# zyansheep/shadow

Hardware: AMD Instinct MI355X
Metric: APSP routing build (s) @10k nodes; packets routed/sec per sim round (lower is better)
Workload: dtype u64+f32; 1 GPU; C3 APSP routing build: 10k-node undirected ring+chords graph, mean degree 8, latency U[1,100] ms (integer us), loss 0 w.p. 0.8 else U(0,0.02); all nodes used; source rows sharded across ranks (each rank keeps its row block; the optional RCCL all-gather of the blocks is timed separately in apsp_detail.allgather_ms); nodes=10000, arcs=79996, parallelism=rows1

## Files before the change

### shadow_amd/csrc/sg_internal.h

```cpp
#pragma once

#include <hip/hip_runtime.h>

#include <cstdint>
#include <cstdio>
#include <new>
#include <stdexcept>
#include <string>
#include <atomic>
#include <deque>
#include <memory>
#include <vector>

#include "../../include/shadow_gpu.h"

namespace sg {

struct Error : std::runtime_error {
  int32_t code;
  uint32_t row, col;
  Error(int32_t c, const std::string& m, uint32_t r = 0, uint32_t k = 0)
      : std::runtime_error(m), code(c), row(r), col(k) {}
};

// ... 182 lines not shown
}

constexpr uint32_t SB_SUB = 8;
constexpr uint32_t SB_CTL_STRIDE = SB_SUB * 4096 + 1;

inline unsigned grid_for(size_t n, unsigned block, unsigned cap = 1u << 20) {
  size_t g = (n + block - 1) / block;
  if (g == 0) g = 1;
  if (g > cap) g = cap;
  return (unsigned)g;
}

void exclusive_scan_u32(sg_ctx* ctx, const uint32_t* d_in, uint32_t* d_out, uint32_t n);

void launch_group_offsets(sg_ctx* ctx, const uint32_t* key, uint32_t n, uint32_t n_groups, uint32_t* off,
                          uint32_t* err);

void copy_to_host(sg_ctx* ctx, void* dst, const void* src, size_t bytes);

char* stage_acquire(sg_ctx* ctx, int slot, size_t bytes);
void stage_release(sg_ctx* ctx, int slot);

void timer_add_work(sg_ctx* ctx, const char* name, double work);
void timer_set_counter(sg_ctx* ctx, const char* name, double work, uint64_t n);

struct TimedLaunch {
  sg_ctx* ctx;
  KernelTimer* timer = nullptr;
  hipEvent_t e0 = nullptr, e1 = nullptr;
  TimedLaunch(sg_ctx* c, const char* name, double work);
  ~TimedLaunch();
};

constexpr uint32_t DENSE_MAX = 4096;
bool sssp_dense_fits(uint32_t n_nodes);
void launch_sssp_dense(sg_ctx* ctx, sg_net* net, const uint32_t* d_used, uint32_t n_used, uint32_t row_begin,
                       uint32_t row_end, uint64_t* out_lat, float* out_loss, uint32_t* sat_row,
                       unsigned long long* work);

bool sssp_bucket_fits(uint32_t n_nodes);
void launch_sssp_bucket(sg_ctx* ctx, sg_net* net, const uint32_t* d_used, uint32_t n_used, uint32_t row_begin,
                        uint32_t row_end, uint64_t* out_lat, float* out_loss, uint32_t* sat_row,
                        unsigned long long* work, unsigned long long* diag);

constexpr int SSSP_KB_MAX = 8;
constexpr uint32_t SSSP_UB_EXACT = 0x80000000u;
bool sssp_lds_fits(uint32_t n_nodes);

struct SsspChainDesc {
  uint32_t* claim;
  const uint32_t* rel;
  const uint8_t* phase_of;
  const uint32_t* pos;
  uint32_t exact, check_rows;
};

struct SsspLdsLaunch {
  const uint32_t* d_used = nullptr;
  uint32_t n_used = 0, row_begin = 0, row_end = 0;
  uint64_t* out_lat = nullptr;
  float* out_loss = nullptr;
  uint32_t* sat_row = nullptr;
  uint32_t delta = 0;
  unsigned long long* work = nullptr;
  unsigned long long* diag = nullptr;
  const uint32_t* blk_rows = nullptr;
  uint32_t n_blk = 0;
  const uint32_t* ub_row = nullptr;
  const uint32_t* ub_w = nullptr;
  const uint32_t* plan_ctl = nullptr;
  int plan_ph = 0;
  uint32_t* plan_ctr = nullptr;
  uint32_t* done = nullptr;
  const SsspChainDesc* chain = nullptr;
};
void launch_sssp_lds(sg_ctx* ctx, const sg_net* net, const SsspLdsLaunch& l);

void ensure_csc(sg_ctx* ctx, sg_net* net);
std::string node_name(const sg_net* net, uint32_t idx);
void launch_zero2(sg_ctx* ctx, uint32_t* a, uint32_t na, uint32_t* b, uint32_t nb);

constexpr int WORK_SHARDS = 64;
void shortest_paths_slab(sg_ctx* ctx, sg_net* net, const uint32_t* d_used, uint32_t n_used, uint32_t row_begin,
                         uint32_t row_end, uint64_t* out_lat, float* out_loss);
void run_wide(sg_ctx* ctx, sg_net* net, const uint32_t* d_used, uint32_t n_used, const std::vector<uint32_t>& rows,
              uint32_t out_row0, uint64_t* out_lat, float* out_loss);

struct SsspDevPlan {
  int n_phase = 0;
  uint32_t* list = nullptr;
  uint32_t* ub_row = nullptr;
  uint32_t* ub_w = nullptr;
  uint32_t* ctl = nullptr;
  uint32_t* ctr = nullptr;
  const SsspChainDesc* chain = nullptr;
  bool landmarks = false;
  unsigned rows_grid = 0;
};
constexpr int SSSP_PHASES_MAX = 6;
SsspDevPlan sssp_device_plan(sg_ctx* ctx, sg_net* net, const uint32_t* d_used, uint32_t n_used, uint32_t row_begin,
                             uint32_t row_end, int n_phase, int kb, bool exact, int hops, uint32_t n_land,
                             uint32_t* zero_rows = nullptr, uint32_t* zero_rows2 = nullptr, bool chain = false,
                             bool chain_exact = false);
const SsspChainDesc* sssp_plain_rel(sg_ctx* ctx, const sg_net* net, const uint32_t* d_used, uint32_t row_begin,
                                    uint32_t row_end, uint32_t* zero_rows, uint32_t* claim, uint32_t* zero_ctr,
                                    bool chain_exact);
void sssp_landmark_bounds(sg_ctx* ctx, const SsspDevPlan& p, uint32_t n_used, uint32_t row_begin,
                          const uint64_t* out_lat, const uint32_t* sat_row, int kb);

}
```

### shadow_amd/csrc/sg_plan.hip

```cpp
#include <algorithm>
#include <cstdlib>
#include <vector>

#include "sg_device.h"
#include "sg_internal.h"
#include "sg_knobs.h"

namespace sg {

__global__ void k_plan_rel(const uint32_t* __restrict__ used, uint32_t row_begin, uint32_t rows,
                           uint32_t* __restrict__ rel, uint8_t* __restrict__ jn, uint32_t* __restrict__ zero_rows,
                           uint32_t* __restrict__ zero_rows2, uint32_t* __restrict__ zero_ctr,
                           SsspChainDesc* __restrict__ desc, SsspChainDesc desc_val) {
  const uint32_t r = blockIdx.x * blockDim.x + threadIdx.x;
  if (zero_ctr && r < 2) zero_ctr[r] = 0;
  if (desc && r == 0) *desc = desc_val;
  if (r >= rows) return;
  rel[used[row_begin + r]] = r;
  if (jn) jn[r] = 0;
  if (zero_rows) zero_rows[r] = 0;
  if (zero_rows2) zero_rows2[r] = 0;
}

constexpr uint32_t PL_OOB = 0x80000000u;
// ... 346 lines not shown
    const uint32_t m = min<uint32_t>(fcnt[wv][cur], PB_FMAX);
    if (!m) break;
    uint32_t carry = 0;
    for (uint32_t e0 = 0; e0 < m; e0 += 64) {
      const uint32_t e = e0 + lane;
      const uint32_t d = e < m ? out_off[fx[wv][cur][e] + 1] - out_off[fx[wv][cur][e]] : 0u;
      const uint32_t incl = wave_incl_sum(d);
      if (e < m) fpre[wv][e] = carry + incl - d;
      carry += __builtin_amdgcn_readlane(incl, 63);
    }
    if (lane == 0) {
      fpre[wv][m] = carry;
      fcnt[wv][cur ^ 1] = 0;
    }
    __builtin_amdgcn_fence(__ATOMIC_RELEASE, "wavefront");
    __builtin_amdgcn_wave_barrier();
    __builtin_amdgcn_fence(__ATOMIC_ACQUIRE, "wavefront");
    for (uint32_t tt = lane; tt < carry; tt += 64) {
      uint32_t lo = 0, hi = m;
      while (hi - lo > 1) {
        const uint32_t mid = (lo + hi) / 2;
        if (fpre[wv][mid] <= tt) lo = mid;
        else hi = mid;
      }
      visit(out_off[fx[wv][cur][lo]] + (tt - fpre[wv][lo]), fw[wv][cur][lo], level, cur ^ 1);
    }
    cur ^= 1;
  }
  for (int k = 0; k < kb; k++) {
    uint64_t mk = t[0];
    for (int d = 32; d > 0; d >>= 1) mk = min(mk, (uint64_t)__shfl_xor((unsigned long long)mk, d));
    if (mk == ~0ull) break;
    const uint32_t q = (uint32_t)mk & 0x7FFFFFFFu;
    if (lane == 0) {
      orow[k] = (row_begin + q) | ((mk >> 63) ? 0u : SSSP_UB_EXACT);
      ow[k] = (uint32_t)(mk >> 31);
    }
#pragma unroll
    for (int j = 0; j < PB_LIST; j++)
      if (((uint32_t)t[j] & 0x7FFFFFFFu) == q) t[j] = ~0ull;
#pragma unroll
    for (int p = 0; p < PB_LIST; p++)
#pragma unroll
      for (int j = 0; j + 1 < PB_LIST; j++) {
        const uint64_t lo = min(t[j], t[j + 1]), hi = max(t[j], t[j + 1]);
        t[j] = lo;
        t[j + 1] = hi;
      }
  }
}

SsspDevPlan sssp_device_plan(sg_ctx* ctx, sg_net* net, const uint32_t* d_used, uint32_t n_used, uint32_t row_begin,
                             uint32_t row_end, int n_phase, int kb, bool exact, int hops, uint32_t n_land,
                             uint32_t* zero_rows, uint32_t* zero_rows2, bool chain, bool chain_exact) {
  (void)n_used;
  const uint32_t n = net->n_nodes, rows = row_end - row_begin;
  n_phase = std::max(2, std::min(SSSP_PHASES_MAX - (n_land ? 1 : 0), n_phase));
  const size_t nl = rows, nb = (size_t)rows * SSSP_KB_MAX;
  const size_t words = nl + 2 * nb + 4 * SSSP_PHASES_MAX + n + 2 * (size_t)rows + 2 * ((rows + 3) / 4) +
                       (sizeof(SsspChainDesc) + 8) / 4;
  uint32_t* w = ctx->r_plan.get<uint32_t>(words);
  SsspDevPlan p;
  p.n_phase = n_phase;
  p.list = w;
  p.ub_row = p.list + nl;
  p.ub_w = p.ub_row + nb;
  p.ctl = p.ub_w + nb;
  p.ctr = p.ctl + 2 * SSSP_PHASES_MAX;
  uint32_t* rel = p.ctr + 2 * SSSP_PHASES_MAX;
  uint32_t* gain = rel + n;
  uint32_t* pos = gain + rows;
  uint8_t* jn = (uint8_t*)(pos + rows);
  uint8_t* phase_of = jn + (rows + 3) / 4 * 4;
  SsspChainDesc* desc = (SsspChainDesc*)(((uintptr_t)(phase_of + (rows + 3) / 4 * 4) + 7) & ~(uintptr_t)7);
  const SsspChainDesc desc_val{zero_rows2, rel, phase_of, pos, chain_exact ? 1u : 0u, 0u};
  if (chain) p.chain = desc;
  hipStream_t st = ctx->stream;
  {
    TimedLaunch tl(ctx, "plan_sets", 0.0);
    if (rows != n) SG_HIP(hipMemsetAsync(rel, 0xff, (size_t)n * 4, st));
    const unsigned g = grid_for(rows, 256);
    hipLaunchKernelGGL(k_plan_rel, dim3(g), dim3(256), 0, st, d_used, row_begin, rows, rel, jn, zero_rows, zero_rows2,
                       (uint32_t*)nullptr, chain ? desc : (SsspChainDesc*)nullptr, desc_val);
    if (net->directed) ensure_csc(ctx, net);
    const uint32_t* in_off = net->directed ? net->in_off : net->out_off;
    const uint32_t* in_idx = net->directed ? net->in_src : net->out_arc;
    const uint32_t in_stride = net->directed ? 1u : 3u;
    for (int ph = 0; ph + 1 < n_phase; ph++) {
      hipLaunchKernelGGL(k_vote_gain, dim3(g), dim3(256), 0, st, in_off, in_idx, in_stride, d_used, row_begin, rows,
                         rel, jn, gain);
      hipLaunchKernelGGL(k_vote_name, dim3(g), dim3(256), 0, st, net->out_off, net->out_arc, d_used, row_begin, rows,
                         rel, jn, gain, ph);
    }
    if (n_land) {
      hipLaunchKernelGGL(k_plan_landmarks<1024>, dim3(1), dim3(1024), 0, st, jn, rows, n_land);
      n_phase += 1;
      p.n_phase = n_phase;
      p.landmarks = true;
      p.rows_grid = grid_for(rows, 256);
    }
    hipLaunchKernelGGL(k_plan_lists<1024>, dim3(1), dim3(1024), 0, st, jn, rows, row_begin, n_phase, phase_of, p.list,
                       pos, p.ctl, p.ctr);
    SG_CHECK_LAUNCH();
  }
  {
    TimedLaunch tl(ctx, "plan_bounds", 0.0);
    hipLaunchKernelGGL(k_plan_bounds, dim3((rows + PB_WAVES - 1) / PB_WAVES), dim3(PB_WAVES * 64), 0, ctx->stream,
                       net->out_off, net->out_arc, d_used, rel, phase_of, p.list, rows, row_begin,
                       std::max(1, std::min(SSSP_KB_MAX, kb)), exact ? 1 : 0, std::max(1, std::min(3, hops)),
                       p.ub_row, p.ub_w);
    SG_CHECK_LAUNCH();
  }
  if (knob_int("SG_PLAN_DIAG", 0) != 0) {
    uint32_t h[2 * SSSP_PHASES_MAX];
    copy_to_host(ctx, h, p.ctl, sizeof(h));
    fprintf(stderr, "[plan] %u rows:", rows);
    for (int ph = 0; ph < n_phase; ph++) fprintf(stderr, " %u", h[2 * ph + 1]);
    fprintf(stderr, "\n");
  }
  return p;
}

const SsspChainDesc* sssp_plain_rel(sg_ctx* ctx, const sg_net* net, const uint32_t* d_used, uint32_t row_begin,
                                    uint32_t row_end, uint32_t* zero_rows, uint32_t* claim, uint32_t* zero_ctr,
                                    bool chain_exact) {
  const uint32_t n = net->n_nodes, rows = row_end - row_begin;
  const size_t dw = sizeof(SsspChainDesc) / 4;
  uint32_t* w = ctx->r_plan.get<uint32_t>(dw + n);
  SsspChainDesc* desc = (SsspChainDesc*)w;
  uint32_t* rel = w + dw;
  const SsspChainDesc desc_val{claim, rel, nullptr, nullptr, chain_exact ? 1u : 0u, rows != n ? rows : 0u};
  hipLaunchKernelGGL(k_plan_rel, dim3(grid_for(rows, 256)), dim3(256), 0, ctx->stream, d_used, row_begin, rows, rel,
                     (uint8_t*)nullptr, zero_rows, claim, zero_ctr, desc, desc_val);
  SG_CHECK_LAUNCH();
  return desc;
}

}
```

### shadow_amd/csrc/sg_routing.hip

```cpp
#include <algorithm>
#include <cstring>
#include <string>
#include <vector>

#include "sg_device.h"
#include "sg_internal.h"
#include "sg_knobs.h"

namespace sg {

__global__ void k_self_check(const uint32_t* __restrict__ used, uint32_t n_used,
                             const uint32_t* __restrict__ self_cnt,
                             unsigned long long* __restrict__ first) {
  for (uint32_t j = blockIdx.x * blockDim.x + threadIdx.x; j < n_used; j += gridDim.x * blockDim.x) {
    uint32_t c = self_cnt[used[j]];
    if (c != 1) atomicMin(first, ((unsigned long long)j << 1) | (c > 1 ? 1ull : 0ull));
  }
}

__global__ void __launch_bounds__(1024) k_build_finish(const uint32_t* __restrict__ sat, uint32_t rows,
                                                       const uint32_t* __restrict__ used, uint32_t n_used,
                                                       const uint32_t* __restrict__ self_cnt, uint32_t* __restrict__ ret) {
  constexpr int G = 8;
  __shared__ uint32_t s_cnt[16];
// ... 231 lines not shown
}

static void print_bucket_diag(const sg_net* net, uint32_t rows, const unsigned long long* d, double total) {
  const double nb = std::max(1.0, (double)d[0]);
  fprintf(stderr, "[bucket] %u rows: %.1f buckets, %.0f entries, %.2f far steps, %.0f pops in %.0f claims, "
          "%.0f relaxations (%.3f x arcs) per row\n", rows, d[0] / (double)rows, d[1] / (double)rows,
          d[2] / (double)rows, d[3] / (double)rows, d[8] / (double)rows, total / rows,
          total / rows / std::max(1u, net->n_arcs));
  fprintf(stderr, "[bucket] cycles per bucket (thread 0): phase 0 %.0f, phase 1 %.0f, phase 2 %.0f; output per row %.0f\n",
          d[4] / nb, d[5] / nb, d[6] / nb, d[7] / (double)rows);
  fprintf(stderr, "[bucket] band kernel, wave 0 per bucket: offsets %.0f, arcs (with appends) %.0f, appends %.0f, store wait %.0f; "
          "band splits per row %.2f\n", d[9] / nb, d[10] / nb, d[11] / nb, d[12] / nb, d[15] / (double)rows);
  fprintf(stderr, "[bucket] band kernel, thread 0 per bucket in the load step: entry loads %.0f, hash %.0f, barrier wait %.0f\n",
          d[8] / nb, d[13] / nb, d[14] / nb);
  const double ncl = std::max(1.0, (double)d[8]);
  fprintf(stderr, "[bucket] per wave and bucket: load step %.0f cyc, idle %.0f; per claim: to offsets %.0f, to "
          "arcs %.0f (sum over arc rounds), appends %.0f, claim total %.0f\n", d[9] / nb / 4, d[14] / nb / 4,
          d[10] / ncl, d[11] / ncl, d[12] / ncl, d[13] / ncl);
}

static void shortest_paths_bucket(sg_ctx* ctx, sg_net* net, const uint32_t* d_used, uint32_t n_used,
                                  uint32_t row_begin, uint32_t row_end, uint64_t* out_lat, float* out_loss) {
  const bool diag_on = knob_int("SG_BUCKET_DIAG", 0) != 0;
  const uint32_t rows = row_end - row_begin;
  uint32_t* sat = ctx->r_flags.get<uint32_t>(std::max(rows, 1u));
  SG_HIP(hipMemsetAsync(sat, 0, std::max(rows, 1u) * 4ull, ctx->stream));
  unsigned long long* work = ctx->count_work ? ctx->r_work.get<unsigned long long>(WORK_SHARDS + 16) : nullptr;
  unsigned long long* diag = work ? work + WORK_SHARDS : nullptr;
  if (work) SG_HIP(hipMemsetAsync(work, 0, (WORK_SHARDS + 16) * 8, ctx->stream));
  {
    TimedLaunch tl(ctx, "sssp_bucket", 0.0);
    launch_sssp_bucket(ctx, net, d_used, n_used, row_begin, row_end, out_lat, out_loss, sat, work, diag);
  }
  std::vector<uint32_t> wide_rows = finish_rows(ctx, sat, row_begin, rows);
  if (work) {
    unsigned long long w[WORK_SHARDS + 16];
    const double total = read_work(ctx, work, w, 16);
    timer_add_work(ctx, "sssp_bucket", total);
    timer_add_work(ctx, "sssp_bucket_entries", (double)w[WORK_SHARDS + 1]);
    if (diag_on) print_bucket_diag(net, rows, w + WORK_SHARDS, total);
  }
  if (!wide_rows.empty()) run_wide(ctx, net, d_used, n_used, wide_rows, row_begin, out_lat, out_loss);
}

struct LdsKnobs {
  uint32_t delta;
  bool diag;
  bool flagged;
  bool phased;
  int n_phase, kb, hops;
  bool exact;
  uint32_t n_land;
  bool chain;
};
static LdsKnobs lds_knobs(const sg_ctx* ctx, const sg_net* net, uint32_t n_used, uint32_t rows) {
  LdsKnobs k;
  k.delta = (uint32_t)std::min(4294967295.0, std::max(1.0, knob_double("SG_APSP_DELTA", 4294967295.0)));
  k.diag = knob_int("SG_SSSP_DIAG", 0) != 0;
  const int seeds_env = knob_int("SG_SSSP_SEEDS", 1);
  const int flag_env = knob_int("SG_SSSP_FLAGGED", -1);
  const bool few_rows = rows < 6u * (uint32_t)std::max(1, ctx->n_cu);
  k.flagged = seeds_env != 0 && (flag_env == 1 || (flag_env < 0 && rows < n_used && !few_rows));
  k.phased = !k.flagged && seeds_env != 0 && (seeds_env == 2 || rows >= 8u * (uint32_t)ctx->n_cu);
  const bool chain = !knob_off("SG_SSSP_CHAIN") && !net->directed && !k.flagged;
  const uint32_t per_cu = rows / std::max(1, ctx->n_cu);
  k.n_phase = knob_int("SG_SSSP_PHASES", per_cu >= 16 && !chain ? 3 : 2, 2, SSSP_PHASES_MAX);
  k.kb = knob_int("SG_SSSP_BOUNDS", 2, 1, SSSP_KB_MAX);
  k.exact = knob_int("SG_SSSP_EXACT", 1) != 0 && n_used == net->n_nodes;
  k.hops = knob_int("SG_SSSP_HOPS", 3, 1, 3);
  const int land_env = knob_int("SG_SSSP_LANDMARKS", 0);
  k.n_land = net->directed || land_env <= 0 ? 0u : (uint32_t)land_env;
  k.chain = chain;
  return k;
}

static void print_sssp_diag(sg_ctx* ctx, const sg_net* net, const unsigned long long* diag, uint32_t n_diag,
                            uint32_t delta) {
  std::vector<unsigned long long> h((size_t)n_diag * 8);
  copy_to_host(ctx, h.data(), diag, h.size() * 8);
  double a[8] = {0, 0, 0, 0, 0, 0, 0, 0};
  double setup = 0;
  double cn[2] = {0, 0}, cs[2] = {0, 0}, cq[2] = {0, 0};
  for (uint32_t r = 0; r < n_diag; r++) {
    for (int k = 0; k < 8; k++) a[k] += (double)h[(size_t)r * 8 + k];
    const unsigned long long w3 = h[(size_t)r * 8 + 3];
    setup += (double)(w3 >> 24);
    a[3] -= (double)(w3 >> 22 << 22);
    if (h[(size_t)r * 8] == 0) continue;
    const int c = (int)((w3 >> 22) & 1);
    cn[c] += 1;
    cs[c] += (double)(w3 >> 24);
    cq[c] += (double)h[(size_t)r * 8];
  }
  for (int c = 0; c < 2; c++)
    fprintf(stderr, "[sssp] %s rows: %.0f, mean setup %.0f cyc, mean search %.0f cyc\n", c ? "chained" : "unchained",
            cn[c], cs[c] / std::max(1.0, cn[c]), cq[c] / std::max(1.0, cn[c]));
  fprintf(stderr, "[sssp] mean setup (init + bound rows) %.0f cyc of the search\n", setup / n_diag);
  fprintf(stderr, "[sssp] per-wave cycles summed over a row's 16 waves: claim+wait %.0f, pop %.0f, steps %.0f "
          "(per pop: %.0f, %.0f)\n", a[5] / n_diag, a[6] / n_diag, a[7] / n_diag, a[6] / std::max(1.0, a[2]),
          a[7] / std::max(1.0, a[2]));
  fprintf(stderr, "[sssp] delta %u ns, %u rows: mean search %.0f cyc, output %.0f cyc, %.1f wave pops, %.1f buckets, "
          "%.0f relaxations (%.2f x arcs)\n", delta, n_diag, a[0] / n_diag, a[1] / n_diag, a[2] / n_diag,
          a[3] / n_diag, a[4] / n_diag, a[4] / n_diag / std::max(1u, net->n_arcs));
}

static void shortest_paths_lds(sg_ctx* ctx, sg_net* net, const uint32_t* d_used, uint32_t n_used, uint32_t row_begin,
                               uint32_t row_end, uint64_t* out_lat, float* out_loss) {
  hipStream_t st = ctx->stream;
  const uint32_t rows = row_end - row_begin;
  const LdsKnobs k = lds_knobs(ctx, net, n_used, rows);
  uint32_t* sat = ctx->r_flags.get<uint32_t>(2 * (size_t)rows);
  uint32_t* claim = k.chain ? sat + rows : nullptr;
  unsigned long long* work = ctx->count_work ? ctx->r_work.get<unsigned long long>(WORK_SHARDS + 2) : nullptr;
  if (work) SG_HIP(hipMemsetAsync(work, 0, (WORK_SHARDS + 2) * 8, st));
  unsigned long long chained_seen[2] = {0, 0};
  unsigned long long phase_chained[SSSP_PHASES_MAX] = {};
  auto diag_chained = [&](const char* what, int ph) {
    if (!work) return;
    unsigned long long c[2];
    copy_to_host(ctx, c, work + WORK_SHARDS, 16);
    phase_chained[ph] = c[0] - chained_seen[0];
    if (k.diag)
      fprintf(stderr, "[sssp] %s %d: %llu chained rows, %llu with exact seeds\n", what, ph, c[0] - chained_seen[0],
              c[1] - chained_seen[1]);
    chained_seen[0] = c[0];
    chained_seen[1] = c[1];
  };
  auto publish_phases = [&](const SsspDevPlan& plan) {
    if (!work) return;
    uint32_t h[2 * SSSP_PHASES_MAX];
    copy_to_host(ctx, h, plan.ctl, sizeof(h));
    for (int p = 0; p < SSSP_PHASES_MAX; p++) {
      char name[24];
      snprintf(name, sizeof(name), "sssp_phase%d", p);
      const bool on = p < plan.n_phase;
      timer_set_counter(ctx, name, on ? (double)phase_chained[p] : 0.0, on ? h[2 * p + 1] : 0u);
    }
  };
  const uint32_t n_diag = std::min<uint32_t>(rows, 4096);
  unsigned long long* diag = work && k.diag ? ctx->r_misc.get<unsigned long long>((size_t)n_diag * 8) : nullptr;
  if (diag) SG_HIP(hipMemsetAsync(diag, 0, (size_t)n_diag * 64, st));
  SsspLdsLaunch base;
  base.d_used = d_used;
  base.n_used = n_used;
  base.row_begin = row_begin;
  base.row_end = row_end;
  base.out_lat = out_lat;
  base.out_loss = out_loss;
  base.sat_row = sat;
  base.delta = k.delta;
  base.work = work;
  base.diag = diag;
  if (k.flagged) {
    uint32_t* done = ctx->r_done.get<uint32_t>(std::max(rows, 1u));
    const SsspDevPlan plan = sssp_device_plan(ctx, net, d_used, n_used, row_begin, row_end, k.n_phase, k.kb, k.exact,
                                              k.hops, 0u, sat, done);
    SsspLdsLaunch l = base;
    l.blk_rows = plan.list;
    l.n_blk = rows;
    l.ub_row = plan.ub_row;
    l.ub_w = plan.ub_w;
    l.plan_ctr = plan.ctr;
    l.done = done;
    {
      TimedLaunch tl(ctx, "sssp", 0.0);
      launch_sssp_lds(ctx, net, l);
    }
    publish_phases(plan);
  } else if (k.phased) {
    const SsspDevPlan plan =
        sssp_device_plan(ctx, net, d_used, n_used, row_begin, row_end, k.n_phase, k.kb, k.exact, k.hops, k.n_land, sat,
                         claim, claim != nullptr, knob_int("SG_SSSP_EXACT", 1) != 0);
    for (int ph = 0; ph < plan.n_phase; ph++) {
      const bool bounded = ph > 0;
      SsspLdsLaunch l = base;
      l.diag = ph + 1 == plan.n_phase ? diag : nullptr;
      l.blk_rows = plan.list;
      l.n_blk = rows;
      l.ub_row = bounded ? plan.ub_row : nullptr;
      l.ub_w = bounded ? plan.ub_w : nullptr;
      l.plan_ctl = plan.ctl;
      l.plan_ph = ph;
      l.plan_ctr = plan.ctr + 2 * ph;
      l.chain = plan.chain;
      {
        TimedLaunch tl(ctx, bounded ? "sssp_bounded" : "sssp", 0.0);
        launch_sssp_lds(ctx, net, l);
      }
      diag_chained("phase", ph);
      if (ph == 0 && plan.landmarks) sssp_landmark_bounds(ctx, plan, n_used, row_begin, out_lat, sat, k.kb);
    }
    publish_phases(plan);
  } else {
    SsspLdsLaunch l = base;
    l.plan_ctr = ctx->r_items.get<uint32_t>(2);
    if (claim && rows > (uint32_t)ctx->n_cu && !knob_off("SG_SSSP_PERSIST")) {
      l.chain = sssp_plain_rel(ctx, net, d_used, row_begin, row_end, sat, claim, l.plan_ctr,
                               knob_int("SG_SSSP_EXACT", 1) != 0);
    } else {
      launch_zero2(ctx, sat, rows, l.plan_ctr, 2u);
    }
    {
      TimedLaunch tl(ctx, "sssp", 0.0);
      launch_sssp_lds(ctx, net, l);
    }
    diag_chained("launch", 0);
  }
  if (diag) print_sssp_diag(ctx, net, diag, n_diag, k.delta);
  std::vector<uint32_t> wide_rows = finish_rows(ctx, sat, row_begin, rows);
  if (work) {
    unsigned long long w[WORK_SHARDS + 2];
    timer_add_work(ctx, "sssp", read_work(ctx, work, w, 2));
    timer_set_counter(ctx, "sssp_chained", (double)w[WORK_SHARDS], w[WORK_SHARDS + 1]);
  }
  if (!wide_rows.empty()) run_wide(ctx, net, d_used, n_used, wide_rows, row_begin, out_lat, out_loss);
}

static void shortest_paths(sg_ctx* ctx, sg_net* net, const uint32_t* d_used, const uint32_t* h_used,
                           uint32_t n_used, uint32_t row_begin, uint32_t row_end, uint64_t* out_lat,
                           float* out_loss) {
  const bool per_source = knob_int("SG_APSP_LDS", 1) != 0;
  const bool dense_on = knob_int("SG_APSP_DENSE", 1) != 0;
  const int bucket_env = knob_int("SG_APSP_BUCKET", -1);
  const bool sparse = net->n_nodes && net->n_arcs <= 64ull * net->n_nodes;
  const bool arcs_ok = (uint64_t)net->n_arcs * 12 < (1ull << 31);
  if (per_source && dense_on && !sparse && sssp_dense_fits(net->n_nodes))
    shortest_paths_dense(ctx, net, d_used, n_used, row_begin, row_end, out_lat, out_loss);
  else if (per_source && sparse && arcs_ok && bucket_env != 0 && sssp_bucket_fits(net->n_nodes) &&
           (bucket_env == 1 || !sssp_lds_fits(net->n_nodes)))
    shortest_paths_bucket(ctx, net, d_used, n_used, row_begin, row_end, out_lat, out_loss);
  else if (per_source && sparse && sssp_lds_fits(net->n_nodes) && arcs_ok)
    shortest_paths_lds(ctx, net, d_used, n_used, row_begin, row_end, out_lat, out_loss);
  else
    shortest_paths_slab(ctx, net, d_used, n_used, row_begin, row_end, out_lat, out_loss);
}


static void direct_paths(sg_ctx* ctx, sg_net* net, const uint32_t* d_used, const uint32_t* h_used,
                         uint32_t n_used, uint32_t row_begin, uint32_t row_end, uint64_t* out_lat,
                         float* out_loss) {
  hipStream_t st = ctx->stream;
  const uint32_t n = net->n_nodes;
  std::vector<uint32_t> map(n, ~0u);
  for (uint32_t j = 0; j < n_used; j++) map[h_used[j]] = j;
  uint32_t* d_map = ctx->r_map.get<uint32_t>(n);
  SG_HIP(hipMemcpyAsync(d_map, map.data(), (size_t)n * 4, hipMemcpyHostToDevice, st));
  size_t count = (size_t)(row_end - row_begin) * n_used;
  uint32_t* cnt = ctx->r_pair_cnt.get<uint32_t>(count);
  uint32_t* edge = ctx->r_pair_edge.get<uint32_t>(count);
  SG_HIP(hipMemsetAsync(cnt, 0, count * 4, st));
  if (net->n_edges)
    hipLaunchKernelGGL(k_pair_count, dim3(grid_for(net->n_edges, 256, 8192)), dim3(256), 0, st,
                       net->e_src, net->e_dst, net->n_edges, (int)net->directed, d_map, n_used,
                       row_begin, row_end, cnt, edge);
  unsigned long long* first = ctx->r_err.get<unsigned long long>(4);
  SG_HIP(hipMemsetAsync(first, 0xff, 8, st));
  hipLaunchKernelGGL(k_pair_out, dim3(grid_for(count, 256, 65536)), dim3(256), 0, st, cnt, edge,
                     count, n_used, row_begin, net->e_lat, net->e_loss, out_lat, out_loss, first);
  SG_CHECK_LAUNCH();
  unsigned long long h = 0;
  copy_to_host(ctx, &h, first, 8);
  if (h != ~0ull) {
    unsigned long long lin = h >> 1;
    uint32_t i = (uint32_t)(lin / n_used), j = (uint32_t)(lin % n_used);
    std::string a = node_name(net, h_used[i]), b = node_name(net, h_used[j]);
    if (h & 1) throw Error(SG_ERR_MULTI_EDGE, "More than one edge connecting node " + a + " to " + b, i, j);
// ... 213 lines not shown
```

### shadow_amd/csrc/sg_sssp.hip

```cpp
#include <algorithm>
#include <cstdlib>
#include <type_traits>

#include "sg_device.h"
#include "sg_internal.h"
#include "sg_knobs.h"

namespace sg {

constexpr int SSSP_THREADS = 1024;
constexpr int SSSP_WAVES = SSSP_THREADS / 64;
constexpr int SSSP_K = 4;
constexpr int SSSP_KB = SSSP_KB_MAX;
constexpr size_t SSSP_STATIC_LDS = 4 * (8 + SSSP_WAVES) + 16 + SSSP_WAVES * 64 * SSSP_K + 512 + 4 * (3 * SSSP_KB + 1) + 16;

constexpr size_t LDS_PER_CU = 160 * 1024;

constexpr uint64_t FKEY_INF = ((uint64_t)LAT32_SAT << 32) | ((uint64_t)0x3F800000u << 1);
__device__ __forceinline__ uint32_t fkey_lat(uint64_t k) { return (uint32_t)(k >> 32); }
__device__ __forceinline__ uint32_t fkey_loss_bits(uint64_t k) { return ((uint32_t)k >> 1) & 0x7FFFFFFFu; }
__device__ __forceinline__ uint64_t frelax(uint64_t ku, uint32_t edge_lat, float edge_om) {
  const uint32_t lat = __builtin_elementwise_add_sat(fkey_lat(ku), edge_lat);
  const float loss = fold_loss(__uint_as_float(fkey_loss_bits(ku)), edge_om);
  return ((uint64_t)lat << 32) | (uint32_t)((__float_as_uint(loss) << 1) | 1u);
// ... 73 lines not shown
  constexpr int TAIL = 1;
  __shared__ unsigned long long hb;
  __shared__ uint8_t own[NW][64 * SSSP_K];
  __shared__ uint32_t red[NW];
  __shared__ unsigned long long sink[64];
  __shared__ uint32_t s_ub[SSSP_KB][3];
  __shared__ uint32_t s_nub;
  __shared__ uint32_t s_sat;
  if (FLAG && threadIdx.x == 0) s_sat = 0u;

  const int tid = threadIdx.x, lane = tid & 63, wv = tid >> 6;
  constexpr uint32_t OOB = 0x80000000u;
  {
    const __amdgpu_buffer_rsrc_t ro = __builtin_amdgcn_make_buffer_rsrc((void*)out_off, 0, (int)((n + 1) * 4u),
                                                                        0x00020000);
    constexpr int GO = 12;
    for (uint32_t v0 = tid; v0 <= n; v0 += GO * NT) {
      uint32_t to[GO];
#pragma unroll
      for (int g = 0; g < GO; g++) {
        const uint32_t v = v0 + g * NT;
        to[g] = __builtin_amdgcn_raw_buffer_load_b32(ro, v <= n ? v * 4u : OOB, 0, 0);
      }
#pragma unroll
      for (int g = 0; g < GO; g++)
        if (v0 + g * NT <= n) off[v0 + g * NT] = to[g];
    }
  }
  __shared__ uint32_t s_item;
  __shared__ uint32_t s_chain, s_cw, s_psat;
  auto next_listed = [&]() -> uint32_t {
    uint32_t* claim_w = chain_on ? chain_args()->claim : nullptr;
    for (;;) {
      const uint32_t b = atomicAdd(item_ctr, 1u);
      if (!claim_w || b >= n_items) return b;
      const uint32_t r = blk_rows ? blk_rows[b] : row_begin + b;
      if (atomicCAS(&claim_w[r - row_begin], 0u, 1u) == 0u) return b;
    }
  };
  if (item_ctr && tid == 0) {
    s_item = next_listed();
    s_chain = 0u;
    s_psat = 0u;
  }
  for (uint32_t it = 0;; it++) {
    uint32_t bi, chain = 0, chain_w = 0;
    if (item_ctr) {
      __syncthreads();
      bi = s_item;
      if (bi >= n_items) break;
      if (chain_on) {
        chain = s_chain;
        chain_w = s_cw;
        if (chain > 1u && !(chain_args()->exact && !s_psat)) chain = 1u;
      }
    } else {
      if (it) break;
      bi = blockIdx.x;
      if (bi >= n_items) break;
    }
    const bool dg = COUNT && diag && bi < 4096 && tid == 0;
    const unsigned long long c_start = dg ? clock64() : 0;
    uint32_t n_adv = 0, n_pops = 0;
    unsigned long long cyc_claim = 0, cyc_pop = 0, cyc_steps = 0;
    const uint32_t row = blk_rows ? blk_rows[bi] : row_begin + bi;
    const uint32_t src = used[row];
    if (chain) {
      const bool ex = (chain & 2u) != 0;
      for (uint32_t v = tid; v < n; v += NT) {
        const uint64_t kv = key[v];
        const uint64_t l = (uint64_t)fkey_lat(kv) + chain_w;
        uint64_t nk = FKEY_INF;
        if (fkey_lat(kv) != LAT32_SAT && l < LAT32_SAT - 1)
          nk = ex ? (l << 32) | ((uint32_t)kv & ~1u) : ((l + 1) << 32) | ((uint64_t)0x3F800000u << 1);
        key[v] = nk;
      }
      if (COUNT && tid == 0) {
        atomicAdd(&work[WORK_SHARDS], 1ull);
        if (ex) atomicAdd(&work[WORK_SHARDS + 1], 1ull);
      }
    } else {
      for (uint32_t v = tid; v < n; v += NT) key[v] = FKEY_INF;
    }
    for (uint32_t i = tid; i < cap; i += NT) ring[i] = RING_EMPTY;
    for (int i = tid; i < NW * 64 * SSSP_K; i += NT) (&own[0][0])[i] = 0;
    if (tid < 8) ctl[tid] = 0;
    if (tid == 0) hb = 0;
    if (ub_row && tid < 64) {
      const uint32_t e = tid < SSSP_KB ? ub_row[(size_t)bi * SSSP_KB + tid] : ~0u;
      const uint32_t w = tid < SSSP_KB ? ub_w[(size_t)bi * SSSP_KB + tid] : 0u;
      const uint32_t srow = e & ~SSSP_UB_EXACT;
      uint32_t sf;
      if constexpr (FLAG) {
        const __amdgpu_buffer_rsrc_t rd = __builtin_amdgcn_make_buffer_rsrc((void*)done, 0, 0x7FFFFFFF, 0x00020000);
        const uint32_t dn = __builtin_amdgcn_raw_buffer_load_b32(rd, e != ~0u ? (srow - row_begin) * 4u : 0x80000000u,
                                                                 0, SSSP_SC1);
        sf = dn == 1u ? 0u : dn == 2u ? 1u : 2u;
      } else {
        sf = e != ~0u ? sat_row[srow - row_begin] : 2u;
      }
      const bool on = sf != 2u;
      const uint64_t mk = __ballot(on);
      if (on) {
        const int at = __popcll(mk & ((1ull << tid) - 1));
        s_ub[at][0] = srow;
        s_ub[at][1] = w;
        s_ub[at][2] = (e & SSSP_UB_EXACT) && sf == 0u;
      }
      if (tid == 0) s_nub = (uint32_t)__popcll(mk);
    }
    __syncthreads();
    if (ub_row) {
      const int nb = (int)s_nub;
      if (nb) {
        const __amdgpu_buffer_rsrc_t ru = __builtin_amdgcn_make_buffer_rsrc((void*)used, 0, (int)(n_used * 4u),
                                                                            0x00020000);
        constexpr int G = 6;
        for (uint32_t j0 = tid; j0 < n_used; j0 += G * NT) {
          uint32_t vv[G];
          uint64_t m[G], ex[G];
#pragma unroll
          for (int g = 0; g < G; g++) {
            const uint32_t j = j0 + g * NT;
            vv[g] = __builtin_amdgcn_raw_buffer_load_b32(ru, j < n_used ? j * 4u : OOB, 0, 0);
            m[g] = ex[g] = ~0ull;
          }
#pragma unroll 1
          for (int k = 0; k < nb; k += 2) {
            bool on[2], exact[2];
            uint32_t sr[2], w[2];
            __amdgpu_buffer_rsrc_t rl[2], rf[2];
#pragma unroll
// ... 273 lines not shown
    const unsigned long long c_search = dg ? clock64() : 0;

    __syncthreads();
    if (item_ctr && !chain_on) {
      if (tid == 0) s_item = atomicAdd(item_ctr, 1u);
    } else if (item_ctr && wv == NW - 1) {
      uint32_t ll = (uint32_t)lane;
      asm volatile("" : "+v"(ll));
      const SsspChainDesc* cd = chain_args();
      uint32_t* claim_w = cd->claim;
      const uint32_t* rel = cd->rel;
      const uint8_t* phase_of = cd->phase_of;
      const uint32_t* list_pos = cd->pos;
      const uint32_t a0 = off[src], nd = min(off[src + 1] - a0, 64u);
      const bool in = ll < nd;
      const auto r = __builtin_amdgcn_raw_buffer_load_b96(arcs, in ? (a0 + ll) * 12u : OOB, 0, 0);
      const __amdgpu_buffer_rsrc_t rr = __builtin_amdgcn_make_buffer_rsrc((void*)rel, 0, (int)(n * 4u), 0x00020000);
      const uint32_t q = __builtin_amdgcn_raw_buffer_load_b32(rr, in ? r[0] * 4u : OOB, 0, 0);
      bool ok = in && q != ~0u;
      if (const uint32_t vr = cd->check_rows) {
        const __amdgpu_buffer_rsrc_t ru = __builtin_amdgcn_make_buffer_rsrc((void*)used, 0, (int)(n_used * 4u), 0x00020000);
        ok = ok && q < vr;
        const uint32_t back = __builtin_amdgcn_raw_buffer_load_b32(ru, ok ? (row_begin + q) * 4u : OOB, 0, 0);
        ok = ok && back == r[0];
      }
      const __amdgpu_buffer_rsrc_t rp = __builtin_amdgcn_make_buffer_rsrc((void*)phase_of, 0, phase_of ? 0x7FFFFFFF : 0, 0x00020000);
      const __amdgpu_buffer_rsrc_t rc = __builtin_amdgcn_make_buffer_rsrc((void*)claim_w, 0, 0x7FFFFFFF, 0x00020000);
      const __amdgpu_buffer_rsrc_t rl = __builtin_amdgcn_make_buffer_rsrc((void*)list_pos, 0, list_pos ? 0x7FFFFFFF : 0, 0x00020000);
      const uint32_t q_ph = __builtin_amdgcn_raw_buffer_load_b8(rp, ok ? q : OOB, 0, 0);
      const uint32_t q_cl = __builtin_amdgcn_raw_buffer_load_b32(rc, ok ? q * 4u : OOB, 0, SSSP_SC1);
      const uint32_t q_at = __builtin_amdgcn_raw_buffer_load_b32(rl, ok ? q * 4u : OOB, 0, 0);
      const uint32_t base = list_pos ? plan_ctl[2 * plan_ph] : 0u;
      ok = ok && q_cl == 0u && (!phase_of || q_ph == (uint32_t)plan_ph);
      uint64_t sc = ok ? ((uint64_t)(r[2] != 0x3F800000u) << 63) | ((uint64_t)r[1] << 31) | q : ~0ull;
      uint32_t got = 0, nb = ~0u, cf = 0, cw = 0;
      for (;;) {
        uint64_t m = sc;
        for (int d = 32; d > 0; d >>= 1) m = min(m, (uint64_t)__shfl_xor((unsigned long long)m, d));
        if (m == ~0ull) break;
        const uint32_t mq = (uint32_t)m & 0x7FFFFFFFu;
        const int win = __ffsll((long long)__ballot(sc == m)) - 1;
        uint32_t old = 1u;
        if ((int)ll == win) old = atomicCAS(&claim_w[mq], 0u, 1u);
        old = __shfl(old, win);
        if (old == 0u) {
          got = 1u;
          cf = 1u | ((m >> 63) ? 0u : 2u);
          cw = (uint32_t)(m >> 31);
          nb = list_pos ? __shfl(q_at, win) - base : mq;
          break;
        }
        if (ok && q == mq) sc = ~0ull;
      }
      if (lane == 0) {
        s_item = got ? nb : next_listed();
        s_chain = cf;
        s_cw = cw;
      }
    }
    const size_t orow = (size_t)(row - out_row0) * n_used;
    bool sat = false;
    typedef unsigned long long u64x2 __attribute__((ext_vector_type(2)));
    typedef float f32x4 __attribute__((ext_vector_type(4)));
    const __amdgpu_buffer_rsrc_t wl = __builtin_amdgcn_make_buffer_rsrc((void*)(out_lat + orow), 0, 0x7FFFFFFF, 0x00020000);
    const __amdgpu_buffer_rsrc_t wf = __builtin_amdgcn_make_buffer_rsrc((void*)(out_loss + orow), 0, 0x7FFFFFFF, 0x00020000);
    auto st_lat2 = [&](uint32_t j, uint64_t a, uint64_t b) {
      if constexpr (FLAG) {
        typedef uint32_t v4 __attribute__((ext_vector_type(4)));
        __builtin_amdgcn_raw_buffer_store_b128((v4){(uint32_t)a, (uint32_t)(a >> 32), (uint32_t)b, (uint32_t)(b >> 32)},
                                               wl, j * 8u, 0, SSSP_SC1);
      } else {
        __builtin_nontemporal_store((u64x2){a, b}, (u64x2*)&out_lat[orow + j]);
      }
    };
    auto st_loss4 = [&](uint32_t j, float a, float b, float c, float d) {
      if constexpr (FLAG) {
        typedef uint32_t v4 __attribute__((ext_vector_type(4)));
        __builtin_amdgcn_raw_buffer_store_b128((v4){__float_as_uint(a), __float_as_uint(b), __float_as_uint(c),
                                                    __float_as_uint(d)}, wf, j * 4u, 0, SSSP_SC1);
      } else {
        __builtin_nontemporal_store((f32x4){a, b, c, d}, (f32x4*)&out_loss[orow + j]);
      }
    };
    auto entry = [&](uint32_t j, uint64_t& l, float& f) {
      if (j == row) {
        const uint32_t e = self_edge[used[j]];
        l = e_lat[e];
        f = e_loss[e];
      } else {
        const uint64_t kk = key[used[j]];
        sat |= fkey_lat(kk) == LAT32_SAT;
        l = fkey_lat(kk);
        f = __uint_as_float(fkey_loss_bits(kk));
      }
    };
    if (vec_out) {
      constexpr int OU = 4;
      const __amdgpu_buffer_rsrc_t ru = __builtin_amdgcn_make_buffer_rsrc((void*)used, 0, (int)(n_used * 4u),
                                                                          0x00020000);
      uint32_t tt = (uint32_t)tid;
      asm volatile("" : "+v"(tt));
      typedef uint32_t u32x4 __attribute__((ext_vector_type(4)));
      u32x4 uv[OU];
#pragma unroll
      for (int k = 0; k < OU; k++) {
        const uint32_t j = (tt + (uint32_t)k * NT) * 4;
        uv[k] = __builtin_amdgcn_raw_buffer_load_b128(ru, j < n_used ? j * 4u : OOB, 0, 0);
      }
// ... 7 lines not shown
        l = diag ? d_lat : (uint64_t)fkey_lat(kk);
        f = diag ? d_loss : __uint_as_float(fkey_loss_bits(kk));
      };
#pragma unroll
      for (int k = 0; k < OU; k++) {
        const uint32_t j = (tt + (uint32_t)k * NT) * 4;
        if (j < n_used) {
          uint64_t l0, l1, l2, l3;
          float f0, f1, f2, f3;
          cell(j, uv[k][0], l0, f0);
          cell(j + 1, uv[k][1], l1, f1);
          cell(j + 2, uv[k][2], l2, f2);
          cell(j + 3, uv[k][3], l3, f3);
          st_lat2(j, l0, l1);
          st_lat2(j + 2, l2, l3);
          st_loss4(j, f0, f1, f2, f3);
        }
      }
      for (uint32_t j = (tt + OU * NT) * 4; j < n_used; j += NT * 4) {
        uint64_t l0, l1, l2, l3;
        float f0, f1, f2, f3;
        entry(j, l0, f0);
        entry(j + 1, l1, f1);
        entry(j + 2, l2, f2);
        entry(j + 3, l3, f3);
        st_lat2(j, l0, l1);
        st_lat2(j + 2, l2, l3);
        st_loss4(j, f0, f1, f2, f3);
      }
    } else {
      for (uint32_t j = tid; j < n_used; j += NT) {
        uint64_t l;
        float f;
        entry(j, l, f);
        if constexpr (FLAG) {
          __builtin_amdgcn_raw_buffer_store_b64((uint32_t __attribute__((ext_vector_type(2)))){(uint32_t)l,
                                                                                              (uint32_t)(l >> 32)},
                                                wl, j * 8u, 0, SSSP_SC1);
          __builtin_amdgcn_raw_buffer_store_b32(__float_as_uint(f), wf, j * 4u, 0, SSSP_SC1);
        } else {
          out_lat[orow + j] = l;
          out_loss[orow + j] = f;
        }
      }
    }
    if (__any(sat) && lane == 0) {
      sat_row[row - row_begin] = 1u;
      if (FLAG) s_sat = 1u;
      if (chain_on) s_psat = 1u;
    }
    if (dg) {
      diag[bi * 8 + 0] = c_search - c_start;
      diag[bi * 8 + 1] = clock64() - c_search;
      diag[bi * 8 + 3] = n_adv | ((unsigned long long)chain << 22) | ((c_setup - c_start) << 24);
    }
    if constexpr (FLAG) {
      asm volatile("s_waitcnt vmcnt(0)" ::: "memory");
      __syncthreads();
      if (tid == 0) {
        const __amdgpu_buffer_rsrc_t rd = __builtin_amdgcn_make_buffer_rsrc((void*)done, 0, 0x7FFFFFFF, 0x00020000);
        __builtin_amdgcn_raw_buffer_store_b32(s_sat ? 2u : 1u, rd, (row - row_begin) * 4u, 0, SSSP_SC1);
        s_sat = 0u;
      }
    }
    __syncthreads();
  }
wave_exit:;
}

bool sssp_lds_fits(uint32_t n) {
  if (n == 0 || n >= RING_EMPTY) return false;
  return sssp_lds_bytes(n) + SSSP_STATIC_LDS <= LDS_PER_CU;
}

struct SsspKnobs {
  uint32_t claim;
  uint32_t idle_sleep;
  uint32_t lane_deg;
  bool persist;
  uint32_t spin_max;
};
static SsspKnobs sssp_knobs() {
  SsspKnobs k;
  k.claim = (uint32_t)knob_int("SG_SSSP_CLAIM", 64, 1, 64);
  k.idle_sleep = (uint32_t)std::max(0, knob_int("SG_SSSP_SLEEP", 0));
  k.lane_deg = (uint32_t)std::max(0, knob_int("SG_SSSP_LANE_DEG", 64));
  k.persist = !knob_off("SG_SSSP_PERSIST");
  k.spin_max = sssp_spin_max();
  return k;
}

void launch_sssp_lds(sg_ctx* ctx, const sg_net* net, const SsspLdsLaunch& l) {
  const SsspKnobs k = sssp_knobs();
  const uint32_t n = net->n_nodes;
  const size_t lds = sssp_lds_bytes(n);
  if (!sssp_lds_fits(n)) throw Error(SG_ERR_INVALID_ARG, "graph too large for the LDS-resident search");
  if ((uint64_t)net->n_arcs * 12 >= (1ull << 31)) throw Error(SG_ERR_INVALID_ARG, "too many arcs for 32-bit offsets");
  const int vec = l.n_used % 4 == 0 && ((uintptr_t)l.out_lat & 15) == 0 && ((uintptr_t)l.out_loss & 15) == 0;
  const uint32_t rows = l.blk_rows ? l.n_blk : l.row_end - l.row_begin;
  if (!rows) return;
  const bool persist = l.done || (k.persist && (rows > (uint32_t)ctx->n_cu || l.plan_ctl));
  uint32_t* item_ctr = nullptr;
  if (persist && l.plan_ctr) {
    item_ctr = l.plan_ctr;
  } else if (persist) {
    item_ctr = ctx->r_items.get<uint32_t>(2);
    SG_HIP(hipMemsetAsync(item_ctr, 0, 8, ctx->stream));
// ... 29 lines not shown
```

Before: 2.717 ms.

## Extend SSSP row chaining to two-hop neighbours and seed listed rows

When a persistent SSSP block finishes a row and finds no unclaimed direct neighbour row, it now searches neighbours two arcs away for an unclaimed source row and claims it, reusing the current distance array as a seed. If it still falls back to the next listed row, it seeds that row from the current distances when that row's node is already reached. Both aim to reduce the per-row initialisation and search work by warm-starting more rows. The extra gather loads, atomics and a wider claim loop add per-row overhead, and the new paths default on only when the non-phased persistent path is used. Diagnostics are extended to count the new chain kinds.

```diff
diff --git a/shadow_amd/csrc/sg_internal.h b/shadow_amd/csrc/sg_internal.h
--- a/shadow_amd/csrc/sg_internal.h
+++ b/shadow_amd/csrc/sg_internal.h
@@ -258,7 +258,7 @@
   const uint32_t* rel;
   const uint8_t* phase_of;
   const uint32_t* pos;
-  uint32_t exact, check_rows;
+  uint32_t exact, check_rows, reach;
 };
 
 struct SsspLdsLaunch {
@@ -307,10 +307,10 @@
 SsspDevPlan sssp_device_plan(sg_ctx* ctx, sg_net* net, const uint32_t* d_used, uint32_t n_used, uint32_t row_begin,
                              uint32_t row_end, int n_phase, int kb, bool exact, int hops, uint32_t n_land,
                              uint32_t* zero_rows = nullptr, uint32_t* zero_rows2 = nullptr, bool chain = false,
-                             bool chain_exact = false);
+                             bool chain_exact = false, uint32_t chain_reach = 0);
 const SsspChainDesc* sssp_plain_rel(sg_ctx* ctx, const sg_net* net, const uint32_t* d_used, uint32_t row_begin,
                                     uint32_t row_end, uint32_t* zero_rows, uint32_t* claim, uint32_t* zero_ctr,
-                                    bool chain_exact);
+                                    bool chain_exact, uint32_t chain_reach);
 void sssp_landmark_bounds(sg_ctx* ctx, const SsspDevPlan& p, uint32_t n_used, uint32_t row_begin,
                           const uint64_t* out_lat, const uint32_t* sat_row, int kb);
 
diff --git a/shadow_amd/csrc/sg_plan.hip b/shadow_amd/csrc/sg_plan.hip
--- a/shadow_amd/csrc/sg_plan.hip
+++ b/shadow_amd/csrc/sg_plan.hip
@@ -422,7 +422,8 @@
 
 SsspDevPlan sssp_device_plan(sg_ctx* ctx, sg_net* net, const uint32_t* d_used, uint32_t n_used, uint32_t row_begin,
                              uint32_t row_end, int n_phase, int kb, bool exact, int hops, uint32_t n_land,
-                             uint32_t* zero_rows, uint32_t* zero_rows2, bool chain, bool chain_exact) {
+                             uint32_t* zero_rows, uint32_t* zero_rows2, bool chain, bool chain_exact,
+                             uint32_t chain_reach) {
   (void)n_used;
   const uint32_t n = net->n_nodes, rows = row_end - row_begin;
   n_phase = std::max(2, std::min(SSSP_PHASES_MAX - (n_land ? 1 : 0), n_phase));
@@ -443,7 +444,7 @@
   uint8_t* jn = (uint8_t*)(pos + rows);
   uint8_t* phase_of = jn + (rows + 3) / 4 * 4;
   SsspChainDesc* desc = (SsspChainDesc*)(((uintptr_t)(phase_of + (rows + 3) / 4 * 4) + 7) & ~(uintptr_t)7);
-  const SsspChainDesc desc_val{zero_rows2, rel, phase_of, pos, chain_exact ? 1u : 0u, 0u};
+  const SsspChainDesc desc_val{zero_rows2, rel, phase_of, pos, chain_exact ? 1u : 0u, 0u, chain_reach};
   if (chain) p.chain = desc;
   hipStream_t st = ctx->stream;
   {
@@ -493,13 +494,14 @@
 
 const SsspChainDesc* sssp_plain_rel(sg_ctx* ctx, const sg_net* net, const uint32_t* d_used, uint32_t row_begin,
                                     uint32_t row_end, uint32_t* zero_rows, uint32_t* claim, uint32_t* zero_ctr,
-                                    bool chain_exact) {
+                                    bool chain_exact, uint32_t chain_reach) {
   const uint32_t n = net->n_nodes, rows = row_end - row_begin;
   const size_t dw = sizeof(SsspChainDesc) / 4;
   uint32_t* w = ctx->r_plan.get<uint32_t>(dw + n);
   SsspChainDesc* desc = (SsspChainDesc*)w;
   uint32_t* rel = w + dw;
-  const SsspChainDesc desc_val{claim, rel, nullptr, nullptr, chain_exact ? 1u : 0u, rows != n ? rows : 0u};
+  const SsspChainDesc desc_val{claim, rel, nullptr, nullptr, chain_exact ? 1u : 0u, rows != n ? rows : 0u,
+                               chain_reach};
   hipLaunchKernelGGL(k_plan_rel, dim3(grid_for(rows, 256)), dim3(256), 0, ctx->stream, d_used, row_begin, rows, rel,
                      (uint8_t*)nullptr, zero_rows, claim, zero_ctr, desc, desc_val);
   SG_CHECK_LAUNCH();
diff --git a/shadow_amd/csrc/sg_routing.hip b/shadow_amd/csrc/sg_routing.hip
--- a/shadow_amd/csrc/sg_routing.hip
+++ b/shadow_amd/csrc/sg_routing.hip
@@ -307,6 +307,7 @@
   bool exact;
   uint32_t n_land;
   bool chain;
+  uint32_t reach;
 };
 static LdsKnobs lds_knobs(const sg_ctx* ctx, const sg_net* net, uint32_t n_used, uint32_t rows) {
   LdsKnobs k;
@@ -326,6 +327,7 @@
   const int land_env = knob_int("SG_SSSP_LANDMARKS", 0);
   k.n_land = net->directed || land_env <= 0 ? 0u : (uint32_t)land_env;
   k.chain = chain;
+  k.reach = chain ? (uint32_t)knob_int("SG_SSSP_CHAIN_REACH", k.phased ? 0 : 2, 0, 2) : 0u;
   return k;
 }
 
@@ -335,21 +337,22 @@
   copy_to_host(ctx, h.data(), diag, h.size() * 8);
   double a[8] = {0, 0, 0, 0, 0, 0, 0, 0};
   double setup = 0;
-  double cn[2] = {0, 0}, cs[2] = {0, 0}, cq[2] = {0, 0};
+  static const char* const kinds[4] = {"unchained", "chained", "two arcs out", "listed, seeded"};
+  double cn[4] = {0, 0, 0, 0}, cs[4] = {0, 0, 0, 0}, cq[4] = {0, 0, 0, 0};
   for (uint32_t r = 0; r < n_diag; r++) {
     for (int k = 0; k < 8; k++) a[k] += (double)h[(size_t)r * 8 + k];
     const unsigned long long w3 = h[(size_t)r * 8 + 3];
     setup += (double)(w3 >> 24);
-    a[3] -= (double)(w3 >> 22 << 22);
+    a[3] -= (double)(w3 >> 20 << 20);
     if (h[(size_t)r * 8] == 0) continue;
-    const int c = (int)((w3 >> 22) & 1);
+    const int c = (w3 >> 22) & 1 ? 1 + (int)std::min<unsigned long long>((w3 >> 20) & 3, 2) : 0;
     cn[c] += 1;
     cs[c] += (double)(w3 >> 24);
     cq[c] += (double)h[(size_t)r * 8];
   }
-  for (int c = 0; c < 2; c++)
-    fprintf(stderr, "[sssp] %s rows: %.0f, mean setup %.0f cyc, mean search %.0f cyc\n", c ? "chained" : "unchained",
-            cn[c], cs[c] / std::max(1.0, cn[c]), cq[c] / std::max(1.0, cn[c]));
+  for (int c = 0; c < 4; c++)
+    fprintf(stderr, "[sssp] %s rows: %.0f, mean setup %.0f cyc, mean search %.0f cyc\n", kinds[c], cn[c],
+            cs[c] / std::max(1.0, cn[c]), cq[c] / std::max(1.0, cn[c]));
   fprintf(stderr, "[sssp] mean setup (init + bound rows) %.0f cyc of the search\n", setup / n_diag);
   fprintf(stderr, "[sssp] per-wave cycles summed over a row's 16 waves: claim+wait %.0f, pop %.0f, steps %.0f "
           "(per pop: %.0f, %.0f)\n", a[5] / n_diag, a[6] / n_diag, a[7] / n_diag, a[6] / std::max(1.0, a[2]),
@@ -366,20 +369,20 @@
   const LdsKnobs k = lds_knobs(ctx, net, n_used, rows);
   uint32_t* sat = ctx->r_flags.get<uint32_t>(2 * (size_t)rows);
   uint32_t* claim = k.chain ? sat + rows : nullptr;
-  unsigned long long* work = ctx->count_work ? ctx->r_work.get<unsigned long long>(WORK_SHARDS + 2) : nullptr;
-  if (work) SG_HIP(hipMemsetAsync(work, 0, (WORK_SHARDS + 2) * 8, st));
-  unsigned long long chained_seen[2] = {0, 0};
+  unsigned long long* work = ctx->count_work ? ctx->r_work.get<unsigned long long>(WORK_SHARDS + 6) : nullptr;
+  if (work) SG_HIP(hipMemsetAsync(work, 0, (WORK_SHARDS + 6) * 8, st));
+  unsigned long long chained_seen[6] = {0, 0, 0, 0, 0, 0};
   unsigned long long phase_chained[SSSP_PHASES_MAX] = {};
   auto diag_chained = [&](const char* what, int ph) {
     if (!work) return;
-    unsigned long long c[2];
-    copy_to_host(ctx, c, work + WORK_SHARDS, 16);
+    unsigned long long c[6];
+    copy_to_host(ctx, c, work + WORK_SHARDS, sizeof(c));
     phase_chained[ph] = c[0] - chained_seen[0];
     if (k.diag)
-      fprintf(stderr, "[sssp] %s %d: %llu chained rows, %llu with exact seeds\n", what, ph, c[0] - chained_seen[0],
-              c[1] - chained_seen[1]);
-    chained_seen[0] = c[0];
-    chained_seen[1] = c[1];
+      fprintf(stderr, "[sssp] %s %d: %llu chained rows, %llu with exact seeds; two arcs out %llu, %llu; listed rows "
+              "seeded %llu, %llu\n", what, ph, c[0] - chained_seen[0], c[1] - chained_seen[1], c[2] - chained_seen[2],
+              c[3] - chained_seen[3], c[4] - chained_seen[4], c[5] - chained_seen[5]);
+    for (int i = 0; i < 6; i++) chained_seen[i] = c[i];
   };
   auto publish_phases = [&](const SsspDevPlan& plan) {
     if (!work) return;
@@ -425,7 +428,7 @@
   } else if (k.phased) {
     const SsspDevPlan plan =
         sssp_device_plan(ctx, net, d_used, n_used, row_begin, row_end, k.n_phase, k.kb, k.exact, k.hops, k.n_land, sat,
-                         claim, claim != nullptr, knob_int("SG_SSSP_EXACT", 1) != 0);
+                         claim, claim != nullptr, knob_int("SG_SSSP_EXACT", 1) != 0, k.reach);
     for (int ph = 0; ph < plan.n_phase; ph++) {
       const bool bounded = ph > 0;
       SsspLdsLaunch l = base;
@@ -451,7 +454,7 @@
     l.plan_ctr = ctx->r_items.get<uint32_t>(2);
     if (claim && rows > (uint32_t)ctx->n_cu && !knob_off("SG_SSSP_PERSIST")) {
       l.chain = sssp_plain_rel(ctx, net, d_used, row_begin, row_end, sat, claim, l.plan_ctr,
-                               knob_int("SG_SSSP_EXACT", 1) != 0);
+                               knob_int("SG_SSSP_EXACT", 1) != 0, k.reach);
     } else {
       launch_zero2(ctx, sat, rows, l.plan_ctr, 2u);
     }
@@ -464,9 +467,11 @@
   if (diag) print_sssp_diag(ctx, net, diag, n_diag, k.delta);
   std::vector<uint32_t> wide_rows = finish_rows(ctx, sat, row_begin, rows);
   if (work) {
-    unsigned long long w[WORK_SHARDS + 2];
-    timer_add_work(ctx, "sssp", read_work(ctx, work, w, 2));
+    unsigned long long w[WORK_SHARDS + 6];
+    timer_add_work(ctx, "sssp", read_work(ctx, work, w, 6));
     timer_set_counter(ctx, "sssp_chained", (double)w[WORK_SHARDS], w[WORK_SHARDS + 1]);
+    timer_set_counter(ctx, "sssp_reach2", (double)w[WORK_SHARDS + 2], w[WORK_SHARDS + 3]);
+    timer_set_counter(ctx, "sssp_listed", (double)w[WORK_SHARDS + 4], w[WORK_SHARDS + 5]);
   }
   if (!wide_rows.empty()) run_wide(ctx, net, d_used, n_used, wide_rows, row_begin, out_lat, out_loss);
 }
diff --git a/shadow_amd/csrc/sg_sssp.hip b/shadow_amd/csrc/sg_sssp.hip
--- a/shadow_amd/csrc/sg_sssp.hip
+++ b/shadow_amd/csrc/sg_sssp.hip
@@ -149,7 +149,7 @@
       if (chain_on) {
         chain = s_chain;
         chain_w = s_cw;
-        if (chain > 1u && !(chain_args()->exact && !s_psat)) chain = 1u;
+        if ((chain & 2u) && !(chain_args()->exact && !s_psat)) chain &= ~2u;
       }
     } else {
       if (it) break;
@@ -173,8 +173,9 @@
         key[v] = nk;
       }
       if (COUNT && tid == 0) {
-        atomicAdd(&work[WORK_SHARDS], 1ull);
-        if (ex) atomicAdd(&work[WORK_SHARDS + 1], 1ull);
+        const uint32_t kd = chain >> 2;
+        atomicAdd(&work[WORK_SHARDS + 2 * kd], 1ull);
+        if (ex) atomicAdd(&work[WORK_SHARDS + 2 * kd + 1], 1ull);
       }
     } else {
       for (uint32_t v = tid; v < n; v += NT) key[v] = FKEY_INF;
@@ -554,8 +555,86 @@
         }
         if (ok && q == mq) sc = ~0ull;
       }
+      const uint32_t reach = cd->reach;
+      if (!got && reach >= 2u && !ub_row) {
+        const uint32_t b0 = in ? off[r[0]] : 0u;
+        const uint32_t bd = in ? min(off[r[0] + 1] - b0, (uint32_t)LA) : 0u;
+        const __amdgpu_buffer_rsrc_t ru = __builtin_amdgcn_make_buffer_rsrc((void*)used, 0, (int)(n_used * 4u), 0x00020000);
+        const uint32_t vr = cd->check_rows;
+        uint32_t c2[LA], q2[LA];
+        bool ok2[LA];
+#pragma unroll
+        for (int k = 0; k < LA; k++)
+          c2[k] = __builtin_amdgcn_raw_buffer_load_b32(arcs, (uint32_t)k < bd ? (b0 + k) * 12u : OOB, 0, 0);
+#pragma unroll
+        for (int k = 0; k < LA; k++) {
+          q2[k] = __builtin_amdgcn_raw_buffer_load_b32(rr, (uint32_t)k < bd ? c2[k] * 4u : OOB, 0, 0);
+        }
+#pragma unroll
+        for (int k = 0; k < LA; k++) ok2[k] = (uint32_t)k < bd && q2[k] != ~0u && (!vr || q2[k] < vr);
+        if (vr) {
+          uint32_t back[LA];
+#pragma unroll
+          for (int k = 0; k < LA; k++)
+            back[k] = __builtin_amdgcn_raw_buffer_load_b32(ru, ok2[k] ? (row_begin + q2[k]) * 4u : OOB, 0, 0);
+#pragma unroll
+          for (int k = 0; k < LA; k++) ok2[k] = ok2[k] && back[k] == c2[k];
+        }
+        uint32_t ph2[LA], cl2[LA];
+#pragma unroll
+        for (int k = 0; k < LA; k++) {
+          ph2[k] = __builtin_amdgcn_raw_buffer_load_b8(rp, ok2[k] ? q2[k] : OOB, 0, 0);
+          cl2[k] = __builtin_amdgcn_raw_buffer_load_b32(rc, ok2[k] ? q2[k] * 4u : OOB, 0, SSSP_SC1);
+        }
+        uint64_t sc2[LA];
+#pragma unroll
+        for (int k = 0; k < LA; k++) {
+          const uint32_t l2 = ok2[k] ? fkey_lat(key[c2[k]]) : LAT32_SAT;
+          const bool on2 = ok2[k] && cl2[k] == 0u && (!phase_of || ph2[k] == (uint32_t)plan_ph) && l2 != LAT32_SAT;
+          sc2[k] = on2 ? ((uint64_t)l2 << 32) | q2[k] : ~0ull;
+        }
+        for (;;) {
+          uint64_t mine = sc2[0];
+#pragma unroll
+          for (int k = 1; k < LA; k++) mine = min(mine, sc2[k]);
+          uint64_t m = mine;
+          for (int d = 32; d > 0; d >>= 1) m = min(m, (uint64_t)__shfl_xor((unsigned long long)m, d));
+          if (m == ~0ull) break;
+          const uint32_t mq = (uint32_t)m;
+          const int win = __ffsll((long long)__ballot(mine == m)) - 1;
+          uint32_t old = 1u, node = 0u;
+          if ((int)ll == win) {
+            old = atomicCAS(&claim_w[mq], 0u, 1u);
+#pragma unroll
+            for (int k = 0; k < LA; k++)
+              if (sc2[k] == m) node = c2[k];
+          }
+          old = __shfl(old, win);
+          if (old == 0u) {
+            node = __shfl(node, win);
+            got = 1u;
+            cf = 1u | 4u | (fkey_loss_bits(key[node]) == 0u ? 2u : 0u);
+            cw = (uint32_t)(m >> 32);
+            nb = list_pos ? list_pos[mq] - base : mq;
+            break;
+          }
+#pragma unroll
+          for (int k = 0; k < LA; k++)
+            if (sc2[k] != ~0ull && (uint32_t)sc2[k] == mq) sc2[k] = ~0ull;
+        }
+      }
       if (lane == 0) {
-        s_item = got ? nb : next_listed();
+        if (!got) {
+          nb = next_listed();
+          if (reach >= 1u && nb < n_items) {
+            const uint64_t kl = key[used[blk_rows ? blk_rows[nb] : row_begin + nb]];
+            if (fkey_lat(kl) != LAT32_SAT) {
+              cf = 1u | 8u | (fkey_loss_bits(kl) == 0u ? 2u : 0u);
+              cw = fkey_lat(kl);
+            }
+          }
+        }
+        s_item = nb;
         s_chain = cf;
         s_cw = cw;
       }
@@ -669,7 +748,8 @@
     if (dg) {
       diag[bi * 8 + 0] = c_search - c_start;
       diag[bi * 8 + 1] = clock64() - c_search;
-      diag[bi * 8 + 3] = n_adv | ((unsigned long long)chain << 22) | ((c_setup - c_start) << 24);
+      diag[bi * 8 + 3] = n_adv | ((unsigned long long)(chain >> 2) << 20) | ((unsigned long long)(chain & 3u) << 22) |
+                         ((c_setup - c_start) << 24);
     }
     if constexpr (FLAG) {
       asm volatile("s_waitcnt vmcnt(0)" ::: "memory");
```

Result: no change. 2.717 ms (+0.0%).
